# cvxopt/smcp

Measured on AMD Instinct MI355X. Metric: Newton KKT solves/sec, higher is better.
Workload: dtype f64; 1 GPU; synth50k nested block-arrow SDP n=50000, 8073 cliques, m=100; kktsolver=chol, n=50000, cliques=8073, m=100, blkval_doubles=2493568, update_doubles=10689536, parallelism=single

## Files before the change

smcp_amd/build.py:

```python
import os
import shutil
import subprocess
import sys

HERE = os.path.dirname(os.path.abspath(__file__))
CSRC = os.path.join(HERE, "csrc")
LIB = os.path.join(HERE, "libsmcp_amd.so")
SOURCES = ["capi.hip", "symbolic.cpp", "constraints.cpp"]


def _stale():
    if not os.path.exists(LIB):
        return True
    t = os.path.getmtime(LIB)
    for d in os.listdir(CSRC):
        if os.path.getmtime(os.path.join(CSRC, d)) > t:
            return True
    return os.path.getmtime(os.path.join(HERE, "..", "include", "smcp_amd.h")) > t


def build(force=False, verbose=True):
    if not force and not _stale():
        return LIB
    hipcc = shutil.which("hipcc") or "/opt/rocm/bin/hipcc"
    cmd = [hipcc, "--offload-arch=gfx950", "-O3", "-std=c++17", "-fPIC", "-shared",
           "-Wno-unused-result", "-Wno-unused-value", "-pthread", "-o", LIB] + [os.path.join(CSRC, s) for s in SOURCES]
    if os.environ.get("SMCP_STAMPS") == "1":
        cmd.insert(1, "-DSMCP_STAMPS")
    for flag in os.environ.get("SMCP_CXXFLAGS", "").split():
        cmd.insert(1, flag)
    if verbose:
        print(" ".join(cmd), file=sys.stderr)
    subprocess.check_call(cmd)
    return LIB


if __name__ == "__main__":
    build(force="--force" in sys.argv)
```

smcp_amd/csrc/capi.hip:

```cpp
#include <hip/hip_runtime.h>
#include <memory>
#include <unordered_map>

#include <algorithm>
#include <chrono>
#include <cstdio>
#include <cstring>
#include <map>
#include <new>
#include <atomic>
#include <thread>
#include <type_traits>
#include <vector>

#include "../../include/smcp_amd.h"
#include "constraints.hpp"
#include "context.hpp"
#include "hostpar.hpp"
#include "switches.hpp"
#include "front_generic.hip"
#include "front_mfma.hip"
#include "front_large.hip"
#include "front_top.hip"
#include "front_inv.hip"
#include "front_n16.hip"
#include "front_downfam.hip"
#include "front_fam.hip"
#include "front_upfam.hip"
#include "front_cholfam.hip"
#include "front_pinvfam.hip"
#include "front_fam2.hip"
#include "front_lfsp.hip"
#include "front_leafgram.hip"
#include "front_famt.hip"
#include "front_flow.hip"
#include "front_mrc.hip"
#include "front_edm.hip"
#include "front_psd.hip"
#include "front_ceig.hip"
#include "front_ceigw.hip"
#include "front_trmm.hip"
#include "front_syr2k.hip"
#include "front_cdec.hip"
#include "front_symm.hip"
#include "front_lowrank.hip"
#include "front_update.hip"
#include "front_lanczos.hip"

using namespace smcp;

#define HIPCHK(x)                                                                        \
  do {                                                                                   \
    hipError_t e_ = (x);                                                                 \
    if (e_ != hipSuccess) {                                                              \
      fprintf(stderr, "smcp_amd: HIP error %s at %s:%d\n", hipGetErrorString(e_), __FILE__, __LINE__); \
      return SMCP_EHIP;                                                                  \
    }                                                                                    \
  } while (0)

namespace {

enum {
  KID_chol_level = 0, KID_llt_level, KID_pinv_level, KID_gather_level, KID_completion_all,
  KID_hess_up_level, KID_hess_down_level, KID_hess_down_inv_all, KID_hess_up_inv_level, KID_scale_an,
  KID_factor_yaa, KID_trsm_fwd_level, KID_trsm_bwd_level, KID_amap, KID_aadj, KID_scatter_constraints,
  KID_dense_potrf, KID_dense_potrs, KID_vec_axpby, KID_axpby, KID_reduce_cliques, KID_reduce_final,
  KID_hess_up_mfma, KID_hess_down_mfma, KID_chol_mfma, KID_pinv_mfma, KID_prep_lk,
  KID_hess_up_mfma_hbm, KID_hess_down_mfma_hbm, KID_chol_mfma_hbm, KID_pinv_mfma_hbm,
  KID_gram_partial, KID_gram_reduce, KID_hess_up_pad,
  KID_lf_assemble, KID_lf_clear_upd, KID_lf_up1, KID_lf_up2, KID_lf_up3, KID_lf_down1, KID_lf_down2, KID_lf_down3,
// ... 2582 lines not shown
```

smcp_amd/csrc/context.hpp:

```cpp
#pragma once
#include <hip/hip_runtime.h>

#include <cstdint>
#include <functional>
#include <map>
#include <vector>

#include "devmem.hpp"
#include "symbolic.hpp"

namespace smcp {

struct CliqueDesc {
  int64_t blk;
  int64_t upd;
  int64_t updp;
  int64_t rows;
  int64_t rel;
  int32_t nn, na;
  int32_t parent;
  int32_t chbeg, chend;
  int32_t first;
  int32_t pad;
};
// ... 33 lines not shown
struct CompletionWs {
  double* ws = nullptr; int64_t cap = 0;
  int32_t* ints = nullptr; double* xdiag = nullptr; int32_t* list = nullptr;
  double* upd2 = nullptr; double* ext = nullptr;
  int64_t* qptr = nullptr; double* wbuf = nullptr;
  double* cone_sw = nullptr; double* cone_mw = nullptr; double* cone_info = nullptr; double* cone_part = nullptr;
  int32_t* cone_list = nullptr; int32_t* cone_sweeps = nullptr;
  double* wws = nullptr; int64_t wcap = 0; CeigwDesc* wdesc = nullptr; int64_t wdesc_cap = 0;
  CeigwDesc* cone_wdesc = nullptr; int64_t cone_wdesc_cap = 0;
};

struct PsdPlan {
  PsdTask* tasks = nullptr; int32_t* ulist = nullptr;
  double* w = nullptr; int32_t* idx = nullptr; int32_t* ra = nullptr;
};

struct ConstraintBufs {
  int64_t m = 0, cnnz = 0;
  int64_t* cptr = nullptr;
  int64_t* cidx = nullptr;
  double* cval = nullptr;
  double* cwval = nullptr;
  int64_t rnnz = 0;
  int64_t* rpos = nullptr;
  int64_t* rptr = nullptr;
  int32_t* rcon = nullptr;
  double* rval = nullptr;
  double* ustack = nullptr;
  int64_t ustack_cols = 0;
  int32_t* a_r = nullptr;
  int32_t* a_c = nullptr;
  int32_t* s_rloc = nullptr;
  int32_t* s_cloc = nullptr;
  int32_t* dlist = nullptr;
  int32_t* slist = nullptr;
  int32_t* kidx = nullptr;
  int64_t md = 0, ns = 0;
  int32_t* kc_ptr = nullptr;
  int32_t* kc_off = nullptr;
  double* kc_val = nullptr;
  int32_t* kc_ij = nullptr;
  int32_t* fz_no = nullptr; int32_t* fz_slot = nullptr; int32_t* fz_ptr = nullptr; int32_t* fz_pk = nullptr; double* fz_s = nullptr;
  int64_t fz_nfam = 0; bool fz_ok = false;
  double* vbuf = nullptr;
  int64_t vcols = 0;
  double* hd = nullptr;
  int32_t* lg_eptr = nullptr; int32_t* lg_epk = nullptr; double* lg_ew = nullptr; int32_t* lg_remap = nullptr;
  double* lg_tab = nullptr;
  int64_t lg_children = 0;
  bool lg_nochild = false;
  double* gpart = nullptr;
  int64_t gpart_len = 0;
  int64_t* gsl_start = nullptr; int32_t* gsl_len = nullptr; int64_t gsl_cap = 0; int gsl_n = 0;
  int gsl_spw = 0, gsl_early = 0;
  int32_t* lg_list = nullptr; int32_t* lg_slot = nullptr; int64_t lg_cap = 0; int lg_cnt = 0;
  int32_t* scm_owner = nullptr;
  double* qr_ws = nullptr;
  int64_t qr_len = 0;
  bool qr_valid = false;
  double* qrm_ws = nullptr;
  int64_t qrm_len = 0;
  int32_t* rinv = nullptr;
  int64_t rinv_len = 0;
  double* res_ws = nullptr;
  int64_t res_len = 0;
  void release(DevLedger& mem) {
    dev_free(mem, cptr, cidx, cval, cwval, rpos, rptr, rcon, rval, ustack, a_r, a_c, s_rloc, s_cloc, dlist, slist, kidx);
    dev_free(mem, kc_ptr, kc_off, kc_val, kc_ij, fz_no, fz_slot, fz_ptr, fz_pk, fz_s, vbuf, hd);
    dev_free(mem, lg_eptr, lg_epk, lg_ew, lg_remap, lg_tab, scm_owner, qr_ws, qrm_ws, gpart, gsl_start, gsl_len, lg_list, lg_slot);
    dev_free(mem, rinv, res_ws);
    *this = ConstraintBufs();
  }
};
struct RhsWorkspaces {
  int64_t max_rhs = 0;
  double* upd = nullptr;
  double* updp = nullptr;
  double* tmp = nullptr;
  void release(DevLedger& mem) { dev_free(mem, upd, updp, tmp); *this = RhsWorkspaces(); }
};

struct DenseChol {
  double* ws = nullptr; int64_t cap = 0;
  struct { const void* A = nullptr; int64_t n = 0; } factored;
  struct { double* H = nullptr; int64_t n = 0, ld = 0; hipStream_t stream = nullptr; } pending;
};

struct DeviceCtx : ConstraintBufs, RhsWorkspaces {
  DevLedger mem;
  int device = -1;
  int ncu = 256;
  CliqueDesc* cl = nullptr;
  int32_t* rowidx = nullptr;
  int32_t* relidx = nullptr;
  int32_t* chidx = nullptr;
  int32_t* levidx = nullptr;
  int32_t* lev2idx = nullptr;
  int64_t* gp_tptr = nullptr;
  int32_t* gp_tgt = nullptr;
  int64_t* gp_cptr = nullptr;
  int32_t* gp_src = nullptr;
  const void* lk_tag_L = nullptr;
  const void* lk_tag_Y = nullptr;
  const void* yaa_tag = nullptr;
  const void* fac_tag = nullptr;
  bool fac_partial = false;
  const void* faci_tag = nullptr;
  double* lfd = nullptr;
  int32_t* lev3idx = nullptr;
  int64_t nI_total = 0, nII_total = 0;
  int nnmaxII_all = 0, namaxII_all = 0;
  double* lfd_dense = nullptr;
  double* lk = nullptr;
  double* yaa = nullptr;
  double* fac = nullptr;
  double* faci = nullptr;
  int64_t* tmpptr = nullptr;
  int64_t tmplen = 0;
  double* red = nullptr;
  int* info = nullptr;
  unsigned long long* fp = nullptr; int* fp_bad = nullptr;
  int* info_host = nullptr;
// ... 150 lines not shown
```

smcp_amd/csrc/front_mfma.hip:

```cpp
#include <hip/hip_runtime.h>

namespace smcp {

typedef double d4 __attribute__((ext_vector_type(4)));

template <class FA, class FB, class FC>
__device__ inline void wg_mma(int M, int N, int Kd, FA A, FB B, FC store, bool lower_only = false, int rot = 0) {
  const int lane = threadIdx.x & 63, nw = blockDim.x >> 6;
  const int wave = ((threadIdx.x >> 6) + nw - (rot % nw)) % nw;
  const int mt = (M + 15) >> 4, nt = (N + 15) >> 4;
  const int l15 = lane & 15, kq = lane >> 4;
  for (int t = wave; t < mt * nt; t += nw) {
    const int tm = t % mt, tn = t / mt;
    if (lower_only && tm < tn) continue;
    const int m = tm * 16 + l15, nb = tn * 16 + l15;
    d4 acc = {0.0, 0.0, 0.0, 0.0};
    constexpr int KU = 2;
    for (int k0 = 0; k0 < Kd; k0 += 4 * KU) {
      double av[KU], bv[KU];
#pragma unroll
      for (int u = 0; u < KU; ++u) {
        const int k = k0 + 4 * u + kq;
        const bool kin = k < Kd;
        av[u] = (kin && m < M) ? A(m, k) : 0.0;
        bv[u] = (kin && nb < N) ? B(k, nb) : 0.0;
      }
#pragma unroll
      for (int u = 0; u < KU; ++u)
        if (k0 + 4 * u < Kd) acc = __builtin_amdgcn_mfma_f64_16x16x4f64(bv[u], av[u], acc, 0, 0, 0);
    }
#pragma unroll
    for (int r = 0; r < 4; ++r) {
      const int n = tn * 16 + kq + 4 * r;
      if (m < M && n < N) store(m, n, acc[r]);
    }
  }
}

template <int UNR, class LoadF, class UseF>
__device__ inline void batched_loop(int begin, int end, int step, LoadF load, UseF use) {
  for (int e0 = begin; e0 < end; e0 += step * UNR) {
    decltype(load(0)) v[UNR];
#pragma unroll
    for (int u = 0; u < UNR; ++u) {
      const int e = e0 + u * step;
      if (e < end) v[u] = load(e);
    }
#pragma unroll
    for (int u = 0; u < UNR; ++u) {
      const int e = e0 + u * step;
      if (e < end) use(e, v[u]);
    }
  }
// ... 1126 lines not shown
  int tms[MAXT], tns[MAXT];
  const int ntile = DIAG ? mti * (mti + 1) / 2 : mti * mtj;
#pragma unroll
  for (int i = 0; i < MAXT; ++i) {
    int p = wave + 4 * i;
    if (p >= ntile) { tms[i] = -1; tns[i] = 0; continue; }
    if (DIAG) { int tm = 0; while (p > tm) { p -= tm + 1; ++tm; } tms[i] = tm; tns[i] = p; }
    else { tms[i] = p % mti; tns[i] = p / mti; }
  }
  d4 acc[MAXT];
#pragma unroll
  for (int i = 0; i < MAXT; ++i) acc[i] = d4{0.0, 0.0, 0.0, 0.0};
  for (int e = threadIdx.x; e < (DIAG ? 1 : 2) * GRAM_KS * GRAM_LD; e += 256) smem[e] = 0.0;
  const int64_t e_begin = e_lo + (int64_t)blockIdx.x * chunk, e_end = min(e_hi, e_begin + chunk);
  const double* const la = sA + kq * GRAM_LD + l15;
  const double* const lb = sB + kq * GRAM_LD + l15;
  for (int64_t e0 = e_begin; e0 < e_end; e0 += GRAM_KS) {
    __syncthreads();
    {
      const int64_t e = e0 + lane;
      const bool ein = e < e_end;
      const double swe = ein ? sw[e] : 0.0;
      batched_loop<16>(wave, ni, 4, [=](int c) { return ein ? G[(int64_t)(ci0 + c) * ldg + e] : 0.0; },
                       [=](int c, double v) { sA[lane * GRAM_LD + c] = swe != 0.0 ? v * swe : 0.0; });
      if (!DIAG)
        batched_loop<16>(wave, nj, 4, [=](int c) { return ein ? G[(int64_t)(cj0 + c) * ldg + e] : 0.0; },
                         [=](int c, double v) { sB[lane * GRAM_LD + c] = swe != 0.0 ? v * swe : 0.0; });
    }
    __syncthreads();
#pragma unroll
    for (int i = 0; i < MAXT; ++i) {
      if (tms[i] < 0) continue;
      const double* const pa = la + 16 * tms[i];
      const double* const pb = lb + 16 * tns[i];
      d4 a = acc[i];
#pragma unroll
      for (int s2 = 0; s2 < GRAM_KS / 4; ++s2)
        a = __builtin_amdgcn_mfma_f64_16x16x4f64(pb[s2 * 4 * GRAM_LD], pa[s2 * 4 * GRAM_LD], a, 0, 0, 0);
      acc[i] = a;
    }
  }
  double* out = partial + ((int64_t)blk * nchunk_total + coff + blockIdx.x) * (int64_t)(64 * 256);
#pragma unroll
  for (int i = 0; i < MAXT; ++i) {
    if (tms[i] < 0) continue;
    const int t = tms[i] + tns[i] * mti;
#pragma unroll
    for (int r = 0; r < 4; ++r) out[(int64_t)t * 256 + (kq + 4 * r) * 16 + l15] = acc[i][r];
  }
}

template <int NT, int NW>
__global__ void __launch_bounds__(64 * NW, (NW == 16 ? 2 : 1)) k_gram_diag128(const double* G, int64_t ldg, int m, const int64_t* sl_start,
                                                      const int32_t* sl_len, int nsl, int spw,
                                                      const double* sw, double* partial, int coff,
                                                      int nchunk_total, int skip) {
  extern __shared__ __attribute__((aligned(16))) double smem[];
  double* const sA = smem;
  const int ni = m;
  const int mti = (ni + 15) >> 4;
  const int lane = threadIdx.x & 63, l15 = lane & 15, kq = lane >> 4;
  const int wave = __builtin_amdgcn_readfirstlane(threadIdx.x >> 6);
  constexpr int NC = GRAM_BLK / NW;
  int tms[NT], tns[NT];
  bool tv[NT];
  const int ntl = mti * (mti + 1) / 2;
#pragma unroll
  for (int i = 0; i < NT; ++i) {
    int p = wave + NW * i, tm = 0;
    tv[i] = p < ntl;
    if (!tv[i]) p = 0;
    while (p > tm) { p -= tm + 1; ++tm; }
    tms[i] = tm; tns[i] = p;
  }
  d4 acc[NT];
#pragma unroll
  for (int i = 0; i < NT; ++i) acc[i] = d4{0.0, 0.0, 0.0, 0.0};
  for (int e = threadIdx.x; e < GRAM_BLK * GRAM_LDK; e += 64 * NW) sA[e] = 0.0;
  const int s_begin = (int)blockIdx.x * spw, s_end = min(nsl, s_begin + spw);
  double pre[NC], pre_sw = 0.0;
  int64_t dstart = 0;
  int dlen = 0;
  auto window = [&](int s0) {
    const int s = s0 + lane;
    dstart = s < s_end ? sl_start[s] : 0;
    dlen = s < s_end ? sl_len[s] : 0;
  };
  auto fetch = [&](int s) {
    const int i = (s - s_begin) & 63;
    const int64_t e0 = ((int64_t)__builtin_amdgcn_readlane((int)(dstart >> 32), i) << 32) | (uint32_t)__builtin_amdgcn_readlane((int)dstart, i);
    const int len = __builtin_amdgcn_readlane(dlen, i);
    const int64_t e = e0 + lane;
    const bool ein = lane < len;
    pre_sw = ein ? sw[e] : 0.0;
#pragma unroll
    for (int j = 0; j < NC; ++j) {
      const int cc = wave + NW * j;
      pre[j] = (ein && cc < ni) ? ((skip & 2) ? 1.0 : G[(int64_t)cc * ldg + e]) : 0.0;
    }
  };
  if (s_begin < s_end) { window(s_begin); fetch(s_begin); }
  const double* const lbase = sA + l15 * GRAM_LDK + kq;
  const double* pa[NT];
  const double* pb[NT];
#pragma unroll
  for (int i = 0; i < NT; ++i) { pa[i] = lbase + 16 * GRAM_LDK * tms[i]; pb[i] = lbase + 16 * GRAM_LDK * tns[i]; }
  for (int sl = s_begin; sl < s_end; ++sl) {
    lds_barrier();
#pragma unroll
    for (int j = 0; j < NC; ++j) {
      const int cc = wave + NW * j;
      if (cc < ni) sA[cc * GRAM_LDK + lane] = pre_sw != 0.0 ? pre[j] * pre_sw : 0.0;
    }
    lds_barrier();
    if (sl + 1 < s_end) {
      if (((sl + 1 - s_begin) & 63) == 0) window(sl + 1);
      fetch(sl + 1);
    }
    if (!(skip & 1))
#pragma unroll
    for (int i = 0; i < NT; i += 2) {
      if (!tv[i]) continue;
      const bool two = (i + 1 < NT) && tv[(i + 1 < NT) ? i + 1 : i];
      d4 a0 = acc[i], a1 = acc[(i + 1 < NT) ? i + 1 : i];
      if (two) {
#pragma unroll
        for (int s2 = 0; s2 < GRAM_KS / 4; ++s2) {
          a0 = __builtin_amdgcn_mfma_f64_16x16x4f64(pb[i][s2 * 4], pa[i][s2 * 4], a0, 0, 0, 0);
          a1 = __builtin_amdgcn_mfma_f64_16x16x4f64(pb[(i + 1 < NT) ? i + 1 : i][s2 * 4], pa[(i + 1 < NT) ? i + 1 : i][s2 * 4], a1, 0, 0, 0);
        }
        acc[(i + 1 < NT) ? i + 1 : i] = a1;
      } else {
#pragma unroll
        for (int s2 = 0; s2 < GRAM_KS / 4; ++s2)
          a0 = __builtin_amdgcn_mfma_f64_16x16x4f64(pb[i][s2 * 4], pa[i][s2 * 4], a0, 0, 0, 0);
      }
      acc[i] = a0;
    }
  }
  double* out = partial + ((int64_t)coff + blockIdx.x) * (int64_t)(64 * 256);
#pragma unroll
  for (int i = 0; i < NT; ++i) {
    if (!tv[i]) continue;
    const int t = tms[i] + tns[i] * mti;
#pragma unroll
    for (int r = 0; r < 4; ++r) out[(int64_t)t * 256 + (kq + 4 * r) * 16 + l15] = acc[i][r];
  }
}

__global__ void k_gram_reduce(const double* partial, int nchunk, int m, double* H, int64_t ldh, double* part_out) {
  int bi = 0, rem = blockIdx.y;
  while (rem > bi) { rem -= bi + 1; ++bi; }
  const int bj = rem;
  const bool diag = bi == bj;
  const int ci0 = bi * GRAM_BLK, cj0 = bj * GRAM_BLK;
  const int ni = min(GRAM_BLK, m - ci0), nj = min(GRAM_BLK, m - cj0);
  const int mti = (ni + 15) >> 4;
  const int t = blockIdx.x;
  const int tm = t % mti, tn = t / mti;
  if (tn * 16 >= nj || (diag && tm < tn)) return;
  __shared__ double zs[4][256];
  const int idx = threadIdx.x & 255;
  const int z = threadIdx.x >> 8, nz = blockDim.x >> 8;
  const int Z = part_out ? (int)gridDim.z : 1, zz = part_out ? (int)blockIdx.z : 0;
  const int r0 = (int)(((int64_t)nchunk * zz) / Z), r1 = (int)(((int64_t)nchunk * (zz + 1)) / Z);
  const int c0 = r0 + (int)(((int64_t)(r1 - r0) * z) / nz), c1 = r0 + (int)(((int64_t)(r1 - r0) * (z + 1)) / nz);
  const double* p = partial + (int64_t)blockIdx.y * nchunk * (int64_t)(64 * 256) + (int64_t)t * 256 + idx;
  double s8[8] = {0.0, 0.0, 0.0, 0.0, 0.0, 0.0, 0.0, 0.0};
  int c = c0;
  for (; c + 8 <= c1; c += 8) {
#pragma unroll
    for (int q = 0; q < 8; ++q) s8[q] += p[(int64_t)(c + q) * (64 * 256)];
  }
  for (; c < c1; ++c) s8[0] += p[(int64_t)c * (64 * 256)];
  double s = ((s8[0] + s8[1]) + (s8[2] + s8[3])) + ((s8[4] + s8[5]) + (s8[6] + s8[7]));
  if (nz > 1) {
    zs[z & 3][idx] = s;
    __syncthreads();
    if (z) return;
    for (int q = 1; q < nz; ++q) s += zs[q][idx];
  }
  if (part_out) {
    part_out[((int64_t)blockIdx.y * Z + zz) * (int64_t)(64 * 256) + (int64_t)t * 256 + idx] = s;
    return;
  }
  const int i = ci0 + tm * 16 + (idx & 15), j = cj0 + tn * 16 + (idx >> 4);
  if (i < ci0 + ni && j < cj0 + nj) {
    H[i + (int64_t)j * ldh] = s;
    H[j + (int64_t)i * ldh] = s;
  }
}

__global__ void k_fill_sqrt_weights(const CliqueDesc* cl, int nsn, double* sw) {
  for (int k = blockIdx.x; k < nsn; k += gridDim.x) {
    const CliqueDesc d = cl[k];
    const int nn = d.nn, nf = d.nn + d.na;
    for (int e = threadIdx.x; e < nf * nn; e += blockDim.x) {
      int i = e % nf, j = e / nf;
      sw[d.blk + e] = (i == j) ? 1.0 : (i > j ? 1.4142135623730951 : 0.0);
    }
  }
}

__global__ void k_selftest_mma(int M, int N, int Kd, const double* A, const double* B, double* C) {
  wg_mma(M, N, Kd, [=](int m, int kk) { return A[m + kk * M]; }, [=](int kk, int n) { return B[kk + n * Kd]; },
         [=](int m, int n, double acc) { C[m + n * M] = acc; });
}

}
```

smcp_amd/csrc/kkt.hip:

```cpp

namespace {

using namespace smcp;

__global__ void __launch_bounds__(1024) k_amap(int64_t m, const int64_t* cptr, const int64_t* cidx, const double* cwval,
                                               const double* X, int64_t ldx, double* y, int64_t ldy, int64_t pstride) {
  __shared__ double part[16];
  const int lane = threadIdx.x & 63, wave = threadIdx.x >> 6, nthr = blockDim.x;
  const int64_t i = blockIdx.x;
  const int r = blockIdx.y;
  const double* x = X + (int64_t)r * ldx;
  const int64_t c0 = cptr[i], c1 = cptr[i + 1], share = (c1 - c0 + gridDim.z - 1) / gridDim.z;
  const int64_t e0 = c0 + (int64_t)blockIdx.z * share, e1 = e0 + share < c1 ? e0 + share : c1;
  y += (int64_t)blockIdx.z * pstride;
  double acc = 0.0;
  for (int64_t e = e0 + threadIdx.x; e < e1; e += 4 * nthr) {
    double w[4], v[4];
#pragma unroll
    for (int q = 0; q < 4; ++q) {
      const int64_t ee = e + (int64_t)q * nthr;
      w[q] = ee < e1 ? cwval[ee] : 0.0;
      v[q] = ee < e1 ? x[cidx[ee]] : 0.0;
    }
#pragma unroll
// ... 211 lines not shown
  amap_impl(c, X, 0, 1, y, 0, (hipStream_t)stream);
  HIPCHK(end_call(c));
  return 0;
}

int kkt_aadj(csp_ctx* c, const double* y, double* X, void* stream) {
  if (int rc = ready(c)) return rc;
  if (!c->D.m) return SMCP_EINVAL;
  if (int rc = aadj_impl(c, y, X, (hipStream_t)stream)) return rc;
  HIPCHK(end_call(c));
  return 0;
}

static bool use_gram(const csp_ctx* c) {
  static int g = -1;
  if (g < 0) { const char* e = sw_str("SMCP_GRAM"); g = (e && e[0] == '0') ? 0 : 1; }
  return g == 1 && !use_generic(c);
}

static bool leafgram_ok(csp_ctx* c, int64_t mcols);
static int gram_prepare(csp_ctx* c, const double* L, const double* Y, hipStream_t st, bool allow_partial_fac = false) {
  DeviceCtx& D = c->D;
  const int64_t m = D.m, bl = c->S.blklen();
  D.qr_valid = false;
  D.lg_nochild = false;
  HIPCHK(zero_flag(c, st));
  prepare_yaa(c, Y, true, st, false, allow_partial_fac);
  if (int rc = prep_lk_cached(c, L, Y, st)) return rc;
  if (!D.kc_ptr) {
    HIPCHK(hipMemsetAsync(D.ustack, 0, sizeof(double) * m * bl, st));
    for (int64_t jb = 0; jb < m; jb += 65535)
      launch(c, KID_scatter_constraints, k_scatter_constraints, dim3(8, (unsigned)std::min<int64_t>(65535, m - jb)),
             dim3(256), st, jb, D.cptr, D.cidx, D.cval, D.ustack + jb * bl, bl);
  }
  HIPCHK(end_call(c));
  return 0;
}
static std::vector<std::pair<int64_t, int64_t>> gram_merge_ranges(int64_t nranges, const int64_t* ranges) {
  std::vector<std::pair<int64_t, int64_t>> rs;
  for (int64_t q = 0; q < nranges; ++q)
    if (ranges[2 * q + 1] > ranges[2 * q]) rs.push_back({ranges[2 * q], ranges[2 * q + 1]});
  std::sort(rs.begin(), rs.end());
  size_t w = 0;
  for (size_t q = 0; q < rs.size(); ++q) {
    if (w && rs[q].first <= rs[w - 1].second) rs[w - 1].second = std::max(rs[w - 1].second, rs[q].second);
    else rs[w++] = rs[q];
  }
  rs.resize(w);
  return rs;
}
static int64_t gram_chunk_rows(int64_t total) {
  static int64_t minrows = 0;
  if (!minrows) { const char* e = sw_str("SMCP_GRAM_MINCHUNK"); minrows = e ? atoll(e) : 512; if (minrows < GRAM_KS) minrows = GRAM_KS; }
  return std::max<int64_t>(minrows, ((total / 512 + GRAM_KS - 1) / GRAM_KS) * GRAM_KS);
}
static int gram_count_chunks(const std::vector<std::pair<int64_t, int64_t>>& rs, int64_t chunk) {
  int n = 0;
  for (auto& r : rs) n += (int)((r.second - r.first + chunk - 1) / chunk);
  return n;
}
static int gram_reserve(csp_ctx* c, int64_t m, int nchunk, hipStream_t st) {
  DeviceCtx& D = c->D;
  const int nb = (int)((m + GRAM_BLK - 1) / GRAM_BLK), nblk = nb * (nb + 1) / 2;
  const int64_t need = (int64_t)nblk * nchunk * 64 * 256;
  return dev_grow(&D.gpart, &D.gpart_len, need, D.mem, st);
}
static int64_t gram_chunk_rows(int64_t total);
static int gram_tables(csp_ctx* c, const std::vector<std::pair<int64_t, int64_t>>& rs, bool leaf, hipStream_t st, bool early_first = false) {
  DeviceCtx& D = c->D;
  const Symbolic& S = c->S;
  std::vector<int64_t> key;
  key.reserve(2 * rs.size() + 1);
  for (auto& r : rs) { key.push_back(r.first); key.push_back(r.second); }
  key.push_back((leaf ? 1 : 0) | (early_first ? 2 : 0));
  if (key == c->gsl_key && D.gsl_start) return 0;
  std::vector<int64_t> start, late_start;
  std::vector<int32_t> len, late_len, list, slot;
  int nf = 0, nn = 0, na = 0;
  auto add_segment = [&](int64_t lo, int64_t hi) {
    if (!early_first) {
      for (int64_t e = lo; e < hi; e += GRAM_KS) { start.push_back(e); len.push_back((int32_t)std::min<int64_t>(GRAM_KS, hi - e)); }
      return;
    }
    int64_t k = (int64_t)(std::upper_bound(S.blkptr.begin(), S.blkptr.end(), lo) - S.blkptr.begin()) - 1;
    for (int64_t p = lo; p < hi; ++k) {
      const int64_t q = std::min(hi, S.blkptr[k + 1]);
      const bool late = S.level[(size_t)k] >= 2;
      for (int64_t e = p; e < q; e += GRAM_KS) {
        (late ? late_start : start).push_back(e);
        (late ? late_len : len).push_back((int32_t)std::min<int64_t>(GRAM_KS, q - e));
      }
      p = q;
    }
  };
  for (auto& r : rs) {
    if (!leaf) { add_segment(r.first, r.second); continue; }
    int64_t k = (int64_t)(std::upper_bound(S.blkptr.begin(), S.blkptr.end(), r.first) - S.blkptr.begin()) - 1;
    int64_t seg_lo = r.first;
    for (; k < S.nsn && S.blkptr[k] < r.second; ++k) {
      if (c->fam[k] != 1) continue;
      const int64_t b = std::max(S.blkptr[k], r.first), e = std::min(S.blkptr[k + 1], r.second);
      if (b != S.blkptr[k] || e != S.blkptr[k + 1]) return SMCP_EINVAL;
      if (b > seg_lo) add_segment(seg_lo, b);
      seg_lo = e;
      list.push_back((int32_t)k);
      slot.push_back(c->lg_slot_of[(size_t)k]);
      nf = std::max(nf, (int)S.nf(k)); nn = std::max(nn, (int)S.nn(k)); na = std::max(na, (int)S.na(k));
    }
    if (r.second > seg_lo) add_segment(seg_lo, r.second);
  }
  D.gsl_spw = 0; D.gsl_early = 0;
  if (early_first) {
    const int64_t chunk = gram_chunk_rows((int64_t)(start.size() + late_start.size()) * GRAM_KS);
    const int spw = (int)(chunk / GRAM_KS);
    while (start.size() % (size_t)spw) { start.push_back(0); len.push_back(0); }
    D.gsl_spw = spw;
    D.gsl_early = late_start.empty() ? 0 : (int)(start.size() / (size_t)spw);
    start.insert(start.end(), late_start.begin(), late_start.end());
    len.insert(len.end(), late_len.begin(), late_len.end());
  }
  const int64_t nslice = std::max<int64_t>((int64_t)start.size(), 1), nlist = std::max<int64_t>((int64_t)list.size(), 1);
  int64_t cap_len = D.gsl_cap, cap_slot = D.lg_cap;
  if (int rc = dev_grow(&D.gsl_start, &D.gsl_cap, nslice, D.mem, st)) return rc;
  if (int rc = dev_grow(&D.gsl_len, &cap_len, nslice, D.mem, st)) return rc;
  if (int rc = dev_grow(&D.lg_list, &D.lg_cap, nlist, D.mem, st)) return rc;
  if (int rc = dev_grow(&D.lg_slot, &cap_slot, nlist, D.mem, st)) return rc;
  HIPCHK(hipStreamSynchronize(st));
  if (!start.empty()) {
    HIPCHK(hipMemcpy(D.gsl_start, start.data(), start.size() * sizeof(int64_t), hipMemcpyHostToDevice));
    HIPCHK(hipMemcpy(D.gsl_len, len.data(), len.size() * sizeof(int32_t), hipMemcpyHostToDevice));
  }
  if (!list.empty()) {
    HIPCHK(hipMemcpy(D.lg_list, list.data(), list.size() * sizeof(int32_t), hipMemcpyHostToDevice));
    HIPCHK(hipMemcpy(D.lg_slot, slot.data(), slot.size() * sizeof(int32_t), hipMemcpyHostToDevice));
  }
  D.gsl_n = (int)start.size();
  D.lg_cnt = (int)list.size();
  D.lg_nf = nf; D.lg_nn = nn; D.lg_na = na;
  c->gsl_key = key;
  return 0;
}

constexpr int LG_ECAP_MAX = 1024;
static bool leafgram_ok(csp_ctx* c, int64_t mcols) {
  static int on = -1;
  if (on < 0) { const char* e = sw_str("SMCP_LEAFGRAM"); on = (e && e[0] == '0') ? 0 : 1; }
  const DeviceCtx& D = c->D;
  if (!on || !c->leafgram_policy || use_generic(c) || !D.kc_ptr || !D.kc_ij || mcols > GRAM_BLK || mcols < 1 || D.lg_children <= 0) return false;
  if (D.lg_maxent > LG_ECAP_MAX) return false;
  if (c->leafgram_policy < 2 && D.lg_pairs > D.lg_rows * mcols) return false;
  if (!D.lg_eptr || !D.lg_tab) return false;
  const int64_t np = mcols * (mcols + 1) / 2 + 1;
  const int ecap = (int)((std::max<int64_t>(D.lg_maxent, 2) + 1) & ~1);
  return np + leafgram_wave_doubles(D.lg_rec, ecap) <= (int64_t)(LDS_LIMIT / 8);
}

static int leafgram_slots(csp_ctx* c) {
  return c->D.ncu;
}
static int leafgram_partials(csp_ctx* c, int64_t mcols, const int32_t* ids, hipStream_t st, double* part, int* nl) {
  DeviceCtx& D = c->D;
  *nl = 0;
  if (!D.lg_cnt) return 0;
  const int ncu = leafgram_slots(c);
  const int64_t np = mcols * (mcols + 1) / 2;
  const int ecap = (int)((std::max<int64_t>(D.lg_maxent, 2) + 1) & ~1);
  const int wd = leafgram_wave_doubles(D.lg_rec, ecap);
  const int64_t lim = (int64_t)(LDS_LIMIT / 8);
  const int nw = (int)std::max<int64_t>(1, std::min<int64_t>(8, (lim - ((np + 1) & ~1)) / wd));
  const int nwg = (int)std::max<int64_t>(1, std::min<int64_t>(ncu, (D.lg_cnt + nw - 1) / nw));
  LeafGramArgs a;
  a.cl = D.cl; a.list = D.lg_list; a.slot = D.lg_slot; a.cnt = D.lg_cnt; a.LK = D.lk; a.yaa = D.yaa;
  a.tab = D.lg_tab; a.rec = D.lg_rec;
  a.eptr = D.lg_eptr; a.epk = D.lg_epk; a.ew = D.lg_ew; a.remap = ids ? D.lg_remap : nullptr;
  a.nr = (int)mcols; a.ecap = ecap;
  a.part = part; a.info = D.info;
  { static int sk = -1; if (sk < 0) { const char* e = sw_str("SMCP_LGSKIP"); sk = e ? atoi(e) : 0; } a.skip = sk; }
  launch_lds(c, KID_leaf_tables, k_leaf_tables, dim3(D.lg_cnt), dim3(64), (size_t)leaftab_doubles(D.lg_nf, D.lg_nn, D.lg_na) * sizeof(double), st,
             a, D.lg_nf, D.lg_nn, D.lg_na);
  const size_t lds = (size_t)(((np + 1) & ~1) + (int64_t)nw * wd) * sizeof(double);
  const int rt = (D.lg_rec + 63) / 64, et = (ecap + 63) / 64;
  bool ok = false;
#define SMCP_LG_CASE(RT, ET) \
  if (!ok && rt <= RT && et <= ET) { \
    static bool attr = false; \
    if (!attr) attr = hipFuncSetAttribute((const void*)k_leaf_pairs<RT, ET>, hipFuncAttributeMaxDynamicSharedMemorySize, 160 * 1024 - 1024) == hipSuccess; \
    if (!attr) return SMCP_EHIP; \
    launch_lds(c, KID_leaf_gram, k_leaf_pairs<RT, ET>, dim3(nwg), dim3(64 * nw), lds, st, a); \
    ok = true; \
  }
  SMCP_LG_CASE(12, 2) SMCP_LG_CASE(12, 4) SMCP_LG_CASE(24, 2) SMCP_LG_CASE(24, 4) SMCP_LG_CASE(24, 16)
  SMCP_LG_CASE(48, 4) SMCP_LG_CASE(48, 16)
#undef SMCP_LG_CASE
  if (!ok) return SMCP_EINVAL;
  *nl = nwg;
  return 0;
}

static void gram_launch_chunks(csp_ctx* c, int64_t m, int spw, int c0, int c1, int nchunk_total, hipStream_t st) {
  DeviceCtx& D = c->D;
  const int64_t bl = c->S.blklen();
  static int nw = -1;
  if (nw < 0) { const char* e = sw_str("SMCP_GRAM_NW"); nw = (e && e[0] == '4') ? 4 : ((e && e[0] == '8') ? 8 : 16); }
  const int mti = (int)((m + 15) / 16), npw = (mti * (mti + 1) / 2 + nw - 1) / nw;
  static int gskip = -1;
  if (gskip < 0) { const char* e = sw_str("SMCP_GSKIP"); gskip = e ? atoi(e) : 0; }
  const size_t lds = (size_t)GRAM_BLK * GRAM_LDK * sizeof(double);
  const int64_t* ss = D.gsl_start + (int64_t)c0 * spw;
  const int32_t* sl = D.gsl_len + (int64_t)c0 * spw;
  const int nsl = std::min<int>(D.gsl_n - c0 * spw, (c1 - c0) * spw);
  const dim3 grid((unsigned)(c1 - c0), 1);
#define SMCP_GRAM_CASE(N) case N: if (nw == 16) launch_lds(c, KID_gram_diag128, k_gram_diag128<(N <= 3 ? N : 3), 16>, grid, dim3(1024), lds, st, \
               (const double*)D.ustack, bl, (int)m, ss, sl, nsl, spw, (const double*)D.sw, D.gpart, c0, nchunk_total, gskip); \
             else if (nw == 8) launch_lds(c, KID_gram_diag128, k_gram_diag128<(N <= 5 ? N : 5), 8>, grid, dim3(512), lds, st, \
               (const double*)D.ustack, bl, (int)m, ss, sl, nsl, spw, (const double*)D.sw, D.gpart, c0, nchunk_total, gskip); \
             else launch_lds(c, KID_gram_diag128, k_gram_diag128<N, 4>, grid, dim3(256), lds, st, \
               (const double*)D.ustack, bl, (int)m, ss, sl, nsl, spw, (const double*)D.sw, D.gpart, c0, nchunk_total, gskip); break;
  switch (npw) {
    SMCP_GRAM_CASE(1) SMCP_GRAM_CASE(2) SMCP_GRAM_CASE(3) SMCP_GRAM_CASE(4) SMCP_GRAM_CASE(5)
    SMCP_GRAM_CASE(6) SMCP_GRAM_CASE(7) SMCP_GRAM_CASE(8) SMCP_GRAM_CASE(9)
  }
#undef SMCP_GRAM_CASE
}

static int gram_accumulate(csp_ctx* c, int64_t nranges, const int64_t* ranges, double* H, int64_t ldh, hipStream_t st,
                           int64_t mcols = -1, bool leaf = false, const int32_t* ids = nullptr) {
  DeviceCtx& D = c->D;
  const int64_t m = mcols < 0 ? D.m : mcols, bl = c->S.blklen();
  const std::vector<std::pair<int64_t, int64_t>> rs = gram_merge_ranges(nranges, ranges);
  int64_t total = 0;
  for (auto& r : rs) total += r.second - r.first;
  if (total <= 0) {
    HIPCHK(hipMemset2DAsync(H, ldh * sizeof(double), 0, m * sizeof(double), m, st));
    return 0;
  }
  const int nb = (int)((m + GRAM_BLK - 1) / GRAM_BLK);
  const int nblk = nb * (nb + 1) / 2;
  if (nblk == 1) {
    int spw, nchunk, ngram, nl = 0;
    Fork* side = (Fork*)c->side_fork;
    c->side_fork = nullptr;
    bool early_done = false;
    int early = 0;
    if (c->gpre.valid && leaf) {
      spw = c->gpre.spw; nchunk = c->gpre.nchunk; ngram = c->gpre.ngram; nl = c->gpre.nl;
      early_done = c->gpre.early_done; early = c->gpre.early;
    } else {
      if (side) { side->join(); delete side; side = nullptr; }
      if (int rc = gram_tables(c, rs, leaf, st)) return rc;
      const int64_t chunk = gram_chunk_rows((int64_t)D.gsl_n * GRAM_KS);
      spw = (int)(chunk / GRAM_KS);
      nchunk = std::max(1, (D.gsl_n + spw - 1) / spw);
      ngram = D.gsl_n > 0 ? nchunk : 0;
      if (int rc = gram_reserve(c, m, nchunk + (leaf ? leafgram_slots(c) : 0) + GRAM_RZ, st)) return rc;
      if (leaf) { if (int rc = leafgram_partials(c, m, ids, st, D.gpart + (int64_t)ngram * (64 * 256), &nl)) return rc; }
    }
    c->gpre.valid = false; c->gpre.early_done = false;
    static int nw = -1;
    if (nw < 0) { const char* e = sw_str("SMCP_GRAM_NW"); nw = (e && e[0] == '4') ? 4 : ((e && e[0] == '8') ? 8 : 16); }
    const int mti = (int)((m + 15) / 16), npw = (mti * (mti + 1) / 2 + nw - 1) / nw;
    static int gskip = -1;
    if (gskip < 0) { const char* e = sw_str("SMCP_GSKIP"); gskip = e ? atoi(e) : 0; }
    const size_t lds = (size_t)GRAM_BLK * GRAM_LDK * sizeof(double);
    (void)nw; (void)npw; (void)gskip; (void)lds;
    const int c0 = early_done ? early : 0;
    if (D.gsl_n > 0 && nchunk > c0) gram_launch_chunks(c, m, spw, c0, nchunk, nchunk, st);
    if (side) { side->join(); delete side; }
    if (ngram + nl >= 256 && D.gpart_len >= (int64_t)(ngram + nl + GRAM_RZ) * (64 * 256)) {
      double* const stage = D.gpart + (int64_t)(ngram + nl) * (64 * 256);
      launch(c, KID_gram_reduce, k_gram_reduce, dim3(64, 1, GRAM_RZ), dim3(1024), st, (const double*)D.gpart, ngram + nl, (int)m, H, ldh, stage);
// ... 460 lines not shown
```

Measured before the change: 372.4 KKT solves/s.

## Pack only nonzero-weight blkval rows into Gram slices via offset tables

The host-side slice builder now drops block-value entries whose symmetric weight is zero (the strict upper triangle of each clique block) and packs the surviving rows into dense 64-row slices. When a slice's rows are not contiguous, it records a per-lane offset table. The Gram MFMA kernel reads these offsets to gather rows, and it exits once it reaches empty padded slices. This roughly halves the rows streamed and multiplied in the Gram accumulation, at the cost of non-contiguous loads, an extra offset fetch per slice, and a more complex table build.

```diff
diff --git a/smcp_amd/build.py b/smcp_amd/build.py
--- a/smcp_amd/build.py
+++ b/smcp_amd/build.py
@@ -6,7 +6,7 @@
 HERE = os.path.dirname(os.path.abspath(__file__))
 CSRC = os.path.join(HERE, "csrc")
 LIB = os.path.join(HERE, "libsmcp_amd.so")
-SOURCES = ["capi.hip", "symbolic.cpp", "constraints.cpp"]
+SOURCES = ["capi.hip", "symbolic.cpp", "constraints.cpp", "gram_rows.cpp"]
 
 
 def _stale():
diff --git a/smcp_amd/csrc/capi.hip b/smcp_amd/csrc/capi.hip
--- a/smcp_amd/csrc/capi.hip
+++ b/smcp_amd/csrc/capi.hip
@@ -16,6 +16,7 @@
 #include "../../include/smcp_amd.h"
 #include "constraints.hpp"
 #include "context.hpp"
+#include "gram_rows.hpp"
 #include "hostpar.hpp"
 #include "switches.hpp"
 #include "front_generic.hip"
diff --git a/smcp_amd/csrc/context.hpp b/smcp_amd/csrc/context.hpp
--- a/smcp_amd/csrc/context.hpp
+++ b/smcp_amd/csrc/context.hpp
@@ -109,6 +109,7 @@
   double* gpart = nullptr;
   int64_t gpart_len = 0;
   int64_t* gsl_start = nullptr; int32_t* gsl_len = nullptr; int64_t gsl_cap = 0; int gsl_n = 0;
+  int32_t* gsl_off = nullptr; int64_t gsl_off_cap = 0;
   int gsl_spw = 0, gsl_early = 0;
   int32_t* lg_list = nullptr; int32_t* lg_slot = nullptr; int64_t lg_cap = 0; int lg_cnt = 0;
   int32_t* scm_owner = nullptr;
@@ -124,7 +125,7 @@
   void release(DevLedger& mem) {
     dev_free(mem, cptr, cidx, cval, cwval, rpos, rptr, rcon, rval, ustack, a_r, a_c, s_rloc, s_cloc, dlist, slist, kidx);
     dev_free(mem, kc_ptr, kc_off, kc_val, kc_ij, fz_no, fz_slot, fz_ptr, fz_pk, fz_s, vbuf, hd);
-    dev_free(mem, lg_eptr, lg_epk, lg_ew, lg_remap, lg_tab, scm_owner, qr_ws, qrm_ws, gpart, gsl_start, gsl_len, lg_list, lg_slot);
+    dev_free(mem, lg_eptr, lg_epk, lg_ew, lg_remap, lg_tab, scm_owner, qr_ws, qrm_ws, gpart, gsl_start, gsl_len, gsl_off, lg_list, lg_slot);
     dev_free(mem, rinv, res_ws);
     *this = ConstraintBufs();
   }
diff --git a/smcp_amd/csrc/front_mfma.hip b/smcp_amd/csrc/front_mfma.hip
--- a/smcp_amd/csrc/front_mfma.hip
+++ b/smcp_amd/csrc/front_mfma.hip
@@ -1,4 +1,6 @@
 #include <hip/hip_runtime.h>
+
+#include "gram_rows.hpp"
 
 namespace smcp {
 
@@ -1231,7 +1233,7 @@
 
 template <int NT, int NW>
 __global__ void __launch_bounds__(64 * NW, (NW == 16 ? 2 : 1)) k_gram_diag128(const double* G, int64_t ldg, int m, const int64_t* sl_start,
-                                                      const int32_t* sl_len, int nsl, int spw,
+                                                      const int32_t* sl_len, const int32_t* sl_off, int nsl, int spw,
                                                       const double* sw, double* partial, int coff,
                                                       int nchunk_total, int skip) {
   extern __shared__ __attribute__((aligned(16))) double smem[];
@@ -1265,11 +1267,17 @@
     dstart = s < s_end ? sl_start[s] : 0;
     dlen = s < s_end ? sl_len[s] : 0;
   };
+  int noff = 0, nlen = 0;
+  auto offsets = [&](int s) {
+    const int blk = __builtin_amdgcn_readlane(dlen, (s - s_begin) & 63) >> GRAM_ROWS_LEN_BITS;
+    noff = blk ? sl_off[(int64_t)(blk - 1) * GRAM_KS + lane] : lane;
+  };
   auto fetch = [&](int s) {
     const int i = (s - s_begin) & 63;
     const int64_t e0 = ((int64_t)__builtin_amdgcn_readlane((int)(dstart >> 32), i) << 32) | (uint32_t)__builtin_amdgcn_readlane((int)dstart, i);
-    const int len = __builtin_amdgcn_readlane(dlen, i);
-    const int64_t e = e0 + lane;
+    const int len = __builtin_amdgcn_readlane(dlen, i) & ((1 << GRAM_ROWS_LEN_BITS) - 1);
+    nlen = len;
+    const int64_t e = e0 + noff;
     const bool ein = lane < len;
     pre_sw = ein ? sw[e] : 0.0;
 #pragma unroll
@@ -1277,14 +1285,16 @@
       const int cc = wave + NW * j;
       pre[j] = (ein && cc < ni) ? ((skip & 2) ? 1.0 : G[(int64_t)cc * ldg + e]) : 0.0;
     }
+    if (s + 1 < s_end && ((s + 1 - s_begin) & 63) != 0) offsets(s + 1);
   };
-  if (s_begin < s_end) { window(s_begin); fetch(s_begin); }
+  if (s_begin < s_end) { window(s_begin); offsets(s_begin); fetch(s_begin); }
   const double* const lbase = sA + l15 * GRAM_LDK + kq;
   const double* pa[NT];
   const double* pb[NT];
 #pragma unroll
   for (int i = 0; i < NT; ++i) { pa[i] = lbase + 16 * GRAM_LDK * tms[i]; pb[i] = lbase + 16 * GRAM_LDK * tns[i]; }
   for (int sl = s_begin; sl < s_end; ++sl) {
+    if (nlen == 0) break;
     lds_barrier();
 #pragma unroll
     for (int j = 0; j < NC; ++j) {
@@ -1293,7 +1303,7 @@
     }
     lds_barrier();
     if (sl + 1 < s_end) {
-      if (((sl + 1 - s_begin) & 63) == 0) window(sl + 1);
+      if (((sl + 1 - s_begin) & 63) == 0) { window(sl + 1); offsets(sl + 1); }
       fetch(sl + 1);
     }
     if (!(skip & 1))
@@ -1376,7 +1386,8 @@
     const int nn = d.nn, nf = d.nn + d.na;
     for (int e = threadIdx.x; e < nf * nn; e += blockDim.x) {
       int i = e % nf, j = e / nf;
-      sw[d.blk + e] = (i == j) ? 1.0 : (i > j ? 1.4142135623730951 : 0.0);
+      const int w = blkval_weight(i, j);
+      sw[d.blk + e] = w == 1 ? 1.0 : (w == 2 ? 1.4142135623730951 : 0.0);
     }
   }
 }
diff --git a/smcp_amd/csrc/gram_rows.cpp b/smcp_amd/csrc/gram_rows.cpp
--- /dev/null
+++ b/smcp_amd/csrc/gram_rows.cpp
@@ -0,0 +1,109 @@
+#include "gram_rows.hpp"
+
+#include <algorithm>
+
+#include "../../include/smcp_amd.h"
+
+namespace smcp {
+
+namespace {
+
+struct Piece { int64_t start; int32_t len; };
+
+struct Packer {
+  std::vector<int64_t>& start;
+  std::vector<int32_t>& desc;
+  std::vector<int32_t>& off;
+  std::vector<int64_t> row;
+  int64_t rows = 0;
+  bool overflow = false;
+
+  void close() {
+    if (row.empty()) return;
+    const int len = (int)row.size();
+    int32_t block = 0;
+    if (row.back() - row.front() != (int64_t)len - 1) {
+      if (row.back() - row.front() > (int64_t)INT32_MAX) overflow = true;
+      block = (int32_t)(off.size() / GRAM_ROWS_KS) + 1;
+      for (int q = 0; q < GRAM_ROWS_KS; ++q) off.push_back(q < len ? (int32_t)(row[(size_t)q] - row.front()) : 0);
+    }
+    start.push_back(row.front());
+    desc.push_back((int32_t)len | (block << GRAM_ROWS_LEN_BITS));
+    rows += len;
+    row.clear();
+  }
+  void add(int64_t p) {
+    row.push_back(p);
+    if ((int)row.size() == GRAM_ROWS_KS) close();
+  }
+};
+
+}
+
+int build_gram_slices(const Symbolic& S, const std::vector<int64_t>& fam, const std::vector<int32_t>* lg_slot_of,
+                      const std::vector<std::pair<int64_t, int64_t>>& rs, bool leaf, bool early_first, int64_t minrows,
+                      GramSlices& T) {
+  T = GramSlices();
+  std::vector<Piece> early, late;
+  auto add_segment = [&](int64_t lo, int64_t hi) {
+    if (!early_first) {
+      for (int64_t e = lo; e < hi; e += GRAM_ROWS_KS) early.push_back({e, (int32_t)std::min<int64_t>(GRAM_ROWS_KS, hi - e)});
+      return;
+    }
+    int64_t k = (int64_t)(std::upper_bound(S.blkptr.begin(), S.blkptr.end(), lo) - S.blkptr.begin()) - 1;
+    for (int64_t p = lo; p < hi; ++k) {
+      const int64_t q = std::min(hi, S.blkptr[k + 1]);
+      std::vector<Piece>& part = S.level[(size_t)k] >= 2 ? late : early;
+      for (int64_t e = p; e < q; e += GRAM_ROWS_KS) part.push_back({e, (int32_t)std::min<int64_t>(GRAM_ROWS_KS, q - e)});
+      p = q;
+    }
+  };
+  for (auto& r : rs) {
+    if (r.first < 0 || r.second > S.blklen()) return SMCP_EINVAL;
+    if (!leaf) { add_segment(r.first, r.second); continue; }
+    int64_t k = (int64_t)(std::upper_bound(S.blkptr.begin(), S.blkptr.end(), r.first) - S.blkptr.begin()) - 1;
+    int64_t seg_lo = r.first;
+    for (; k < S.nsn && S.blkptr[k] < r.second; ++k) {
+      if (fam[(size_t)k] != 1) continue;
+      const int64_t b = std::max(S.blkptr[k], r.first), e = std::min(S.blkptr[k + 1], r.second);
+      if (b != S.blkptr[k] || e != S.blkptr[k + 1]) return SMCP_EINVAL;
+      if (b > seg_lo) add_segment(seg_lo, b);
+      seg_lo = e;
+      T.list.push_back((int32_t)k);
+      T.slot.push_back(lg_slot_of ? (*lg_slot_of)[(size_t)k] : 0);
+      T.nf = std::max(T.nf, (int)S.nf(k)); T.nn = std::max(T.nn, (int)S.nn(k)); T.na = std::max(T.na, (int)S.na(k));
+    }
+    if (r.second > seg_lo) add_segment(seg_lo, r.second);
+  }
+  int64_t chunk = 0;
+  if (early_first) {
+    chunk = gram_chunk_rows_of((int64_t)(early.size() + late.size()) * GRAM_ROWS_KS, minrows);
+    const size_t spw = (size_t)(chunk / GRAM_ROWS_KS);
+    while (early.size() % spw) early.push_back({0, 0});
+    T.spw = (int)spw;
+    T.early = late.empty() ? 0 : (int)(early.size() / spw);
+    early.insert(early.end(), late.begin(), late.end());
+  } else {
+    chunk = gram_chunk_rows_of((int64_t)early.size() * GRAM_ROWS_KS, minrows);
+  }
+  const size_t spw = (size_t)(chunk / GRAM_ROWS_KS), n = early.size();
+  Packer P{T.start, T.desc, T.off};
+  int64_t k = 0;
+  for (size_t c0 = 0; c0 < n; c0 += spw) {
+    const size_t c1 = std::min(n, c0 + spw);
+    for (size_t s = c0; s < c1; ++s)
+      for (int64_t e = early[s].start; e < early[s].start + early[s].len; ++e) {
+        if (e < S.blkptr[k] || e >= S.blkptr[k + 1]) k = (int64_t)(std::upper_bound(S.blkptr.begin(), S.blkptr.end(), e) - S.blkptr.begin()) - 1;
+        const int64_t b = S.blkptr[k], nf = S.nf(k);
+        if (blkval_weight((e - b) % nf, (e - b) / nf) != 0) P.add(e);
+      }
+    P.close();
+    if (T.start.size() > c1) return SMCP_EINVAL;
+    while (T.start.size() < c1) { T.start.push_back(0); T.desc.push_back(0); }
+  }
+  if (P.overflow) return SMCP_EINVAL;
+  T.rows = P.rows;
+  return 0;
+}
+
+}
diff --git a/smcp_amd/csrc/gram_rows.hpp b/smcp_amd/csrc/gram_rows.hpp
--- /dev/null
+++ b/smcp_amd/csrc/gram_rows.hpp
@@ -0,0 +1,39 @@
+#pragma once
+#include <cstdint>
+#include <utility>
+#include <vector>
+
+#include "symbolic.hpp"
+
+#if defined(__HIPCC__) || defined(__CUDACC__)
+#define SMCP_GRAM_HD __host__ __device__
+#else
+#define SMCP_GRAM_HD
+#endif
+
+namespace smcp {
+
+SMCP_GRAM_HD inline int blkval_weight(int64_t i, int64_t j) { return i == j ? 1 : (i > j ? 2 : 0); }
+
+constexpr int GRAM_ROWS_KS = 64;
+constexpr int GRAM_ROWS_LEN_BITS = 7;
+
+inline int64_t gram_chunk_rows_of(int64_t total, int64_t minrows) {
+  const int64_t r = ((total / 512 + GRAM_ROWS_KS - 1) / GRAM_ROWS_KS) * GRAM_ROWS_KS;
+  return r > minrows ? r : minrows;
+}
+
+struct GramSlices {
+  std::vector<int64_t> start;
+  std::vector<int32_t> desc, off;
+  std::vector<int32_t> list, slot;
+  int nf = 0, nn = 0, na = 0;
+  int spw = 0, early = 0;
+  int64_t rows = 0;
+};
+
+int build_gram_slices(const Symbolic& S, const std::vector<int64_t>& fam, const std::vector<int32_t>* lg_slot_of,
+                      const std::vector<std::pair<int64_t, int64_t>>& rs, bool leaf, bool early_first, int64_t minrows,
+                      GramSlices& T);
+
+}
diff --git a/smcp_amd/csrc/kkt.hip b/smcp_amd/csrc/kkt.hip
--- a/smcp_amd/csrc/kkt.hip
+++ b/smcp_amd/csrc/kkt.hip
@@ -287,7 +287,7 @@
 static int64_t gram_chunk_rows(int64_t total) {
   static int64_t minrows = 0;
   if (!minrows) { const char* e = sw_str("SMCP_GRAM_MINCHUNK"); minrows = e ? atoll(e) : 512; if (minrows < GRAM_KS) minrows = GRAM_KS; }
-  return std::max<int64_t>(minrows, ((total / 512 + GRAM_KS - 1) / GRAM_KS) * GRAM_KS);
+  return gram_chunk_rows_of(total, minrows);
 }
 static int gram_count_chunks(const std::vector<std::pair<int64_t, int64_t>>& rs, int64_t chunk) {
   int n = 0;
@@ -300,6 +300,7 @@
   const int64_t need = (int64_t)nblk * nchunk * 64 * 256;
   return dev_grow(&D.gpart, &D.gpart_len, need, D.mem, st);
 }
+static_assert(GRAM_ROWS_KS == GRAM_KS, "slice length of the table builder");
 static int64_t gram_chunk_rows(int64_t total);
 static int gram_tables(csp_ctx* c, const std::vector<std::pair<int64_t, int64_t>>& rs, bool leaf, hipStream_t st, bool early_first = false) {
   DeviceCtx& D = c->D;
@@ -309,61 +310,28 @@
   for (auto& r : rs) { key.push_back(r.first); key.push_back(r.second); }
   key.push_back((leaf ? 1 : 0) | (early_first ? 2 : 0));
   if (key == c->gsl_key && D.gsl_start) return 0;
-  std::vector<int64_t> start, late_start;
-  std::vector<int32_t> len, late_len, list, slot;
-  int nf = 0, nn = 0, na = 0;
-  auto add_segment = [&](int64_t lo, int64_t hi) {
-    if (!early_first) {
-      for (int64_t e = lo; e < hi; e += GRAM_KS) { start.push_back(e); len.push_back((int32_t)std::min<int64_t>(GRAM_KS, hi - e)); }
-      return;
-    }
-    int64_t k = (int64_t)(std::upper_bound(S.blkptr.begin(), S.blkptr.end(), lo) - S.blkptr.begin()) - 1;
-    for (int64_t p = lo; p < hi; ++k) {
-      const int64_t q = std::min(hi, S.blkptr[k + 1]);
-      const bool late = S.level[(size_t)k] >= 2;
-      for (int64_t e = p; e < q; e += GRAM_KS) {
-        (late ? late_start : start).push_back(e);
-        (late ? late_len : len).push_back((int32_t)std::min<int64_t>(GRAM_KS, q - e));
-      }
-      p = q;
-    }
-  };
-  for (auto& r : rs) {
-    if (!leaf) { add_segment(r.first, r.second); continue; }
-    int64_t k = (int64_t)(std::upper_bound(S.blkptr.begin(), S.blkptr.end(), r.first) - S.blkptr.begin()) - 1;
-    int64_t seg_lo = r.first;
-    for (; k < S.nsn && S.blkptr[k] < r.second; ++k) {
-      if (c->fam[k] != 1) continue;
-      const int64_t b = std::max(S.blkptr[k], r.first), e = std::min(S.blkptr[k + 1], r.second);
-      if (b != S.blkptr[k] || e != S.blkptr[k + 1]) return SMCP_EINVAL;
-      if (b > seg_lo) add_segment(seg_lo, b);
-      seg_lo = e;
-      list.push_back((int32_t)k);
-      slot.push_back(c->lg_slot_of[(size_t)k]);
-      nf = std::max(nf, (int)S.nf(k)); nn = std::max(nn, (int)S.nn(k)); na = std::max(na, (int)S.na(k));
-    }
-    if (r.second > seg_lo) add_segment(seg_lo, r.second);
-  }
-  D.gsl_spw = 0; D.gsl_early = 0;
-  if (early_first) {
-    const int64_t chunk = gram_chunk_rows((int64_t)(start.size() + late_start.size()) * GRAM_KS);
-    const int spw = (int)(chunk / GRAM_KS);
-    while (start.size() % (size_t)spw) { start.push_back(0); len.push_back(0); }
-    D.gsl_spw = spw;
-    D.gsl_early = late_start.empty() ? 0 : (int)(start.size() / (size_t)spw);
-    start.insert(start.end(), late_start.begin(), late_start.end());
-    len.insert(len.end(), late_len.begin(), late_len.end());
-  }
+  static int64_t minrows = 0;
+  if (!minrows) minrows = gram_chunk_rows(0);
+  GramSlices T;
+  if (int rc = build_gram_slices(S, c->fam, &c->lg_slot_of, rs, leaf, early_first, minrows, T)) return rc;
+  const std::vector<int64_t>& start = T.start;
+  const std::vector<int32_t>& len = T.desc;
+  const std::vector<int32_t>& list = T.list;
+  const std::vector<int32_t>& slot = T.slot;
+  const int nf = T.nf, nn = T.nn, na = T.na;
+  D.gsl_spw = T.spw; D.gsl_early = T.early;
   const int64_t nslice = std::max<int64_t>((int64_t)start.size(), 1), nlist = std::max<int64_t>((int64_t)list.size(), 1);
   int64_t cap_len = D.gsl_cap, cap_slot = D.lg_cap;
   if (int rc = dev_grow(&D.gsl_start, &D.gsl_cap, nslice, D.mem, st)) return rc;
   if (int rc = dev_grow(&D.gsl_len, &cap_len, nslice, D.mem, st)) return rc;
+  if (int rc = dev_grow(&D.gsl_off, &D.gsl_off_cap, std::max<int64_t>((int64_t)T.off.size(), 1), D.mem, st)) return rc;
   if (int rc = dev_grow(&D.lg_list, &D.lg_cap, nlist, D.mem, st)) return rc;
   if (int rc = dev_grow(&D.lg_slot, &cap_slot, nlist, D.mem, st)) return rc;
   HIPCHK(hipStreamSynchronize(st));
   if (!start.empty()) {
     HIPCHK(hipMemcpy(D.gsl_start, start.data(), start.size() * sizeof(int64_t), hipMemcpyHostToDevice));
     HIPCHK(hipMemcpy(D.gsl_len, len.data(), len.size() * sizeof(int32_t), hipMemcpyHostToDevice));
+    if (!T.off.empty()) HIPCHK(hipMemcpy(D.gsl_off, T.off.data(), T.off.size() * sizeof(int32_t), hipMemcpyHostToDevice));
   }
   if (!list.empty()) {
     HIPCHK(hipMemcpy(D.lg_list, list.data(), list.size() * sizeof(int32_t), hipMemcpyHostToDevice));
@@ -446,11 +414,11 @@
   const int nsl = std::min<int>(D.gsl_n - c0 * spw, (c1 - c0) * spw);
   const dim3 grid((unsigned)(c1 - c0), 1);
 #define SMCP_GRAM_CASE(N) case N: if (nw == 16) launch_lds(c, KID_gram_diag128, k_gram_diag128<(N <= 3 ? N : 3), 16>, grid, dim3(1024), lds, st, \
-               (const double*)D.ustack, bl, (int)m, ss, sl, nsl, spw, (const double*)D.sw, D.gpart, c0, nchunk_total, gskip); \
+               (const double*)D.ustack, bl, (int)m, ss, sl, (const int32_t*)D.gsl_off, nsl, spw, (const double*)D.sw, D.gpart, c0, nchunk_total, gskip); \
              else if (nw == 8) launch_lds(c, KID_gram_diag128, k_gram_diag128<(N <= 5 ? N : 5), 8>, grid, dim3(512), lds, st, \
-               (const double*)D.ustack, bl, (int)m, ss, sl, nsl, spw, (const double*)D.sw, D.gpart, c0, nchunk_total, gskip); \
+               (const double*)D.ustack, bl, (int)m, ss, sl, (const int32_t*)D.gsl_off, nsl, spw, (const double*)D.sw, D.gpart, c0, nchunk_total, gskip); \
              else launch_lds(c, KID_gram_diag128, k_gram_diag128<N, 4>, grid, dim3(256), lds, st, \
-               (const double*)D.ustack, bl, (int)m, ss, sl, nsl, spw, (const double*)D.sw, D.gpart, c0, nchunk_total, gskip); break;
+               (const double*)D.ustack, bl, (int)m, ss, sl, (const int32_t*)D.gsl_off, nsl, spw, (const double*)D.sw, D.gpart, c0, nchunk_total, gskip); break;
   switch (npw) {
     SMCP_GRAM_CASE(1) SMCP_GRAM_CASE(2) SMCP_GRAM_CASE(3) SMCP_GRAM_CASE(4) SMCP_GRAM_CASE(5)
     SMCP_GRAM_CASE(6) SMCP_GRAM_CASE(7) SMCP_GRAM_CASE(8) SMCP_GRAM_CASE(9)
```

Result: no change. 374.5 KKT solves/s, median of 6 (+0.6%).
